# zhu-xlab/PFST

Measured on AMD Instinct MI355X. Metric: PFST train-step images/s on 1024² IRRG tiles, higher is better.
Workload: dtype f32 (f16x3 split MFMA: two scaled fp16 pieces per operand, three products, fp32 accumulate); 1 GPU; pfst_pots_irrg2vaih_irrg_deeplabv3plus_r50-d8; global_batch=8, per_gpu_batch=8, tile=1024x1024x3, num_classes=6, parallelism=dp1, weights=seeded random init, conv_math=f16x3

## Files before the change

### pfst_amd/csrc/conv_f16x3.hip

```cpp
#include "conv_epilogue.h"
#include "amax.h"
#include "wgrad_launch.h"
#include "weight_jobs.h"
#include <math.h>
#include <stdlib.h>
#include <type_traits>
#include <utility>
#include "../../include/pfst_hip.h"

typedef _Float16 f16x8 __attribute__((ext_vector_type(8)));
typedef float f32x4 __attribute__((ext_vector_type(4)));

namespace {

constexpr int BN = 128;
constexpr int NP = 2;

__global__ __launch_bounds__(256) void absmax_kernel(const float* __restrict__ x, i64 n, i64 plane_stride, int slot_stride,
                                                     float* __restrict__ slots) {
  const float* p = x + (i64)blockIdx.y * plane_stride;
  float m = 0.f;
  const i64 n4 = (((uintptr_t)p & 15) == 0) ? n / 4 : 0;
  for (i64 i = (i64)blockIdx.x * blockDim.x + threadIdx.x; i < n4; i += (i64)gridDim.x * blockDim.x) {
    const float4 v = reinterpret_cast<const float4*>(p)[i];
// ... 218 lines not shown
    if constexpr (ONE) {
      ld_oy = p;
      ld_ox = 0;
    } else {
      ld_oy = ld_pvalid ? p / Wo : 0;
      ld_ox = ld_pvalid ? p - ld_oy * Wo : 0;
    }
    a_voff = (m0 + a_row < M) ? 16u * ((unsigned)a_seg * (unsigned)M + (unsigned)(m0 + a_row)) : OOB;
    a_rsrc = __builtin_amdgcn_make_buffer_rsrc(const_cast<uint4*>(wk4) + (i64)y * KT16 * 2 * NP * M, 0, KT16 * 2 * NP * M * 16, 0x00020000);
    b_rsrc = __builtin_amdgcn_make_buffer_rsrc(const_cast<float*>(in) + (i64)n * in_bs, 0, C * HiWi * 4, 0x00020000);
  };
  auto tap_voff = [&](int tap) -> unsigned {
    if constexpr (ONE) return ld_pvalid ? 4u * ((unsigned)(bt * 16 + kh * 8) * (unsigned)HiWi + (unsigned)ld_oy) : OOB;
    const int ty = tap / ks, tx = tap - ty * ks;
    int sy, sx;
    const bool ok = ld_pvalid & src_coord(ld_oy, ty, ca, cb, cc, cdivv, Hi, sy) & src_coord(ld_ox, tx, ca, cb, cc, cdivv, Wi, sx);
    return ok ? 4u * ((unsigned)(kh * 8) * (unsigned)HiWi + (unsigned)(sy * Wi + sx)) : OOB;
  };

  uint4 areg[2][NA];
  float breg[2][TPT][8];
  pfst_f32x16 acc32[TMW][2];
#pragma unroll
  for (int i = 0; i < TMW; ++i)
#pragma unroll
    for (int j = 0; j < 2; ++j)
#pragma unroll
      for (int r = 0; r < 16; ++r) acc32[i][j][r] = 0.f;

  auto load_b = [&](auto vc, auto setc, unsigned voff, int soff) {
    constexpr int v = decltype(vc)::value, SET = decltype(setc)::value;
    breg[SET][v >> 3][v & 7] = __builtin_bit_cast(float, __builtin_amdgcn_raw_buffer_load_b32(b_rsrc, voff, soff + ((v >> 3) * 16 + (v & 7)) * b_chan, 0));
  };
  auto load_a = [&](auto vc, auto setc, int a_soff) {
    constexpr int v = decltype(vc)::value, SET = decltype(setc)::value;
    areg[SET][v] = __builtin_bit_cast(uint4, __builtin_amdgcn_raw_buffer_load_b128(a_rsrc, a_voff, a_soff + (v / (NA / 2)) * a_tile + (v % (NA / 2)) * a_chunk, 0));
  };
  int tap2 = 0, sidx2 = 0;
  int sidx1 = 0;
  unsigned voff2 = OOB;
  auto advance = [&]() {
    sidx1 = sidx2;
    if (++sidx2 == spt) {
      sidx2 = 0;
      ++tap2;
      if (tap2 < ntaps) {
        voff2 = tap_voff(tap2);
      } else if (CHAIN && tap2 == ntaps && ld_lin + G < total) {
        ld_lin += G;
        set_load_side(ld_lin);
        tap2 = 0;
        voff2 = tap_voff(0);
      } else {
        voff2 = OOB;
      }
    }
  };

  const int eb = amax_exponent(amax_read(in_amax));
  const float sb = __builtin_bit_cast(float, __builtin_amdgcn_readfirstlane(__builtin_bit_cast(int, scale_of(eb))));
  int ea = 0, ea_y = -1;

  auto prologue = [&](int lin) {
    ld_lin = lin;
    set_load_side(lin);
    tap2 = sidx2 = 0;
    voff2 = tap_voff(0);
    static_for<8 * TPT>([&](auto vc) { load_b(vc, std::integral_constant<int, 0>(), voff2, 0); });
    static_for<NA>([&](auto vc) { load_a(vc, std::integral_constant<int, 0>(), 0); });
    advance();
#pragma unroll
    for (int v = 0; v < NA; ++v) As[(v / (NA / 2)) * TILE_A + tid + NT * (v % (NA / 2))] = areg[0][v];
#pragma unroll
    for (int t = 0; t < TPT; ++t) {
      uint4 ph, pl;
      if constexpr (BNL) {
        const float2* cf = reinterpret_cast<const float2*>(bnl_s) + (t + bt) * 16 + kh * 8;
#pragma unroll
        for (int i = 0; i < 8; ++i) breg[0][t][i] = fmaxf(__fmaf_rn(breg[0][t][i], cf[i].x, cf[i].y), 0.f);
      }
      if constexpr (BPACK) unpack8_f16(breg[0][t], ph, pl);
      else split8_f16(breg[0][t], sb, ph, pl);
      Bs[(t + bt) * TILE_B + (0 * 2 + kh) * BN + pix] = ph;
      Bs[(t + bt) * TILE_B + (1 * 2 + kh) * BN + pix] = pl;
    }
    {
      const int soff = sidx2 * chan_step, a_soff = (tap2 * spt + sidx2) * 2 * a_tile;
      static_for<8 * TPT>([&](auto vc) { load_b(vc, std::integral_constant<int, 1>(), voff2, soff); });
      static_for<NA>([&](auto vc) { load_a(vc, std::integral_constant<int, 1>(), a_soff); });
    }
    advance();
    __syncthreads();
  };

  const int l15 = lane & 15, lq = lane >> 4;
  const int a_frag = (lq >> 1) * TILE_A + (lq & 1) * BM + wm0 + l15;
  const int b_frag = (lq >> 1) * TILE_B + (lq & 1) * BN + wn0 + l15;

  const int l31 = lane & 31, lh = lane >> 5;
  auto step32 = [&](auto setn_c, int k) {
    constexpr int SETN = decltype(setn_c)::value, SETL = SETN ^ 1;
    constexpr int CUR = SETL * PAIR_CHUNKS, NXT = SETN * PAIR_CHUNKS;
    f16x8 af[2][TMW][NP], bf[2][2][NP];
    auto rd_a = [&](int t, int i, int pl) { af[t][i][pl] = __builtin_bit_cast(f16x8, As[CUR + t * TILE_A + (pl * 2 + lh) * BM + wm0 + i * 32 + l31]); };
    auto rd_b = [&](int t, int j, int pl) { bf[t][j][pl] = __builtin_bit_cast(f16x8, Bs[CUR + t * TILE_B + (pl * 2 + lh) * BN + wn0 + j * 32 + l31]); };
    constexpr int RG = 2 + TMW;
    auto read_frag = [&](auto rc) {
      constexpr int r = decltype(rc)::value, grp = r / RG, e = r % RG, t = grp & 1, pa = grp < 2 ? 1 : 0, pb = grp < 2 ? 0 : 1;
      if constexpr (e == 0) rd_a(t, 0, pa);
      else if constexpr (e == 1) rd_b(t, 0, pb);
      else if constexpr (e == 2) rd_b(t, 1, pb);
      else rd_a(t, 1, pa);
    };
    const int soff2 = sidx2 * chan_step;
    const int a_soff2 = (tap2 * spt + sidx2) * 2 * a_tile;
    constexpr int PRE = TMW == 2 ? RG : 2 * RG;
    static_for<PRE>([&](auto rc) { read_frag(rc); });
    __builtin_amdgcn_sched_barrier(0);
    SplitF16 s0, s1;
    uint4 cfr[BNL ? 4 : 1];
    const int cf_at = BNL ? sidx1 * 16 + bt * 8 + kh * 4 : 0;
    auto filler = [&](auto sc) {
      constexpr int m = decltype(sc)::value;
      if constexpr (m < 8) {
        if constexpr (TPT == 2) {
          load_b(std::integral_constant<int, 2 * m>(), std::integral_constant<int, SETL>(), voff2, soff2);
          load_b(std::integral_constant<int, 2 * m + 1>(), std::integral_constant<int, SETL>(), voff2, soff2);
        } else {
          load_b(std::integral_constant<int, m>(), std::integral_constant<int, SETL>(), voff2, soff2);
        }
      }
      if constexpr (m >= 8 && m < 8 + NA) As[NXT + ((m - 8) / (NA / 2)) * TILE_A + tid + NT * ((m - 8) % (NA / 2))] = areg[SETN][m - 8];
      if constexpr (BNL && m >= 8 && m < 12) cfr[m - 8] = bnl_s[cf_at + (m - 8)];
      if constexpr (m >= 12) {
        constexpr int SPS = 2 * TPT;
        static_for<SPS>([&](auto kc) {
          constexpr int kk = (m - 12) * SPS + decltype(kc)::value;
          if constexpr (BPACK) {
            if constexpr (kk < 8) unpack_op_f16<kk>(breg[SETN][0], s0);
            else if constexpr (kk < 16 && TPT == 2) unpack_op_f16<kk - 8>(breg[SETN][TPT - 1], s1);
          } else {
            if constexpr (BNL && kk < 24 && kk % 6 < 2) {
              constexpr int e = 2 * (kk / 6) + kk % 6;
              const uint4 c2 = cfr[e >> 1];
              const float sc = __builtin_bit_cast(float, (e & 1) ? c2.z : c2.x), sh = __builtin_bit_cast(float, (e & 1) ? c2.w : c2.y);
              breg[SETN][0][e] = fmaxf(__fmaf_rn(breg[SETN][0][e], sc, sh), 0.f);
            }
            if constexpr (kk < 24) split_op_f16<kk>(breg[SETN][0], sb, s0);
            else split_op_f16<kk - 24>(breg[SETN][TPT - 1], sb, s1);
          }
        });
      }
      if constexpr (m >= 12 && m < 12 + NA) load_a(std::integral_constant<int, m - 12>(), std::integral_constant<int, SETL>(), a_soff2);
      if constexpr (m == 18 && TPT == 2) {
        Bs[NXT + (0 * 2 + kh) * BN + pix] = make_uint4(s0.h[0], s0.h[1], s0.h[2], s0.h[3]);
        Bs[NXT + (1 * 2 + kh) * BN + pix] = make_uint4(s0.l[0], s0.l[1], s0.l[2], s0.l[3]);
      }
      if constexpr (m == 23 && TPT == 2) {
        Bs[NXT + TILE_B + (0 * 2 + kh) * BN + pix] = make_uint4(s1.h[0], s1.h[1], s1.h[2], s1.h[3]);
        Bs[NXT + TILE_B + (1 * 2 + kh) * BN + pix] = make_uint4(s1.l[0], s1.l[1], s1.l[2], s1.l[3]);
      }
      if constexpr (m == 23 && TPT == 1) {
        Bs[NXT + bt * TILE_B + (0 * 2 + kh) * BN + pix] = make_uint4(s0.h[0], s0.h[1], s0.h[2], s0.h[3]);
        Bs[NXT + bt * TILE_B + (1 * 2 + kh) * BN + pix] = make_uint4(s0.l[0], s0.l[1], s0.l[2], s0.l[3]);
      }
    };
    static_for<12 * TMW>([&](auto mc) {
      constexpr int m = decltype(mc)::value;
      constexpr int prod = m / (4 * TMW), rem = m % (4 * TMW), t = rem / (2 * TMW), i = (rem >> 1) % TMW, j = rem & 1;
      constexpr int pa = prod == 0 ? 1 : 0, pb = prod == 1 ? 1 : 0;
      acc32[i][j] = __builtin_amdgcn_mfma_f32_32x32x16_f16(af[t][i][pa], bf[t][j][pb], acc32[i][j], 0, 0, 0);
      if constexpr (PRE + m < 4 * RG) read_frag(std::integral_constant<int, PRE + m>());
      if constexpr (TMW == 2) {
        filler(std::integral_constant<int, m>());
      } else {
        filler(std::integral_constant<int, 2 * m>());
        filler(std::integral_constant<int, 2 * m + 1>());
      }
      __builtin_amdgcn_sched_barrier(0);
    });
    advance();
    __syncthreads();
  };
  auto epilogue = [&](int lin) {
    int bx, by, y, n;
    decode(lin, bx, by, y, n);
    if (y != ea_y) {
      ea = amax_exponent(amax_read(w_amax + (i64)y * PFST_AMAX_SUB));
      ea_y = y;
    }
    const int p0 = bx * BN, m0 = by * BM;
    float* const outn = out + (i64)n * out_bs;
    const float* const gsrc = gate.g ? gate.g + (i64)n * gate.g_bs : nullptr;
    const unsigned long long* const gmask = gate.g ? gate.mask + (i64)n * M * (P >> 6) : nullptr;
    const float ua = unscale_of(ea), ub = unscale_of(eb);
    {
#pragma unroll
      for (int i = 0; i < TMW; ++i)
#pragma unroll
        for (int j = 0; j < 2; ++j)
#pragma unroll
          for (int r = 0; r < 16; ++r) acc32[i][j][r] = acc32[i][j][r] * ua * ub;
      if constexpr (BNB != 0) {
        static_assert(PAIR_CHUNKS * sizeof(uint4) >= (NT / 64) * PFST_ROWSUM_LDS_FLOATS * sizeof(float), "epilogue scratch must fit into one pair buffer");
        conv_epilogue<2, 2, WAVES_N, BN, BNB, true>(acc32, outn, bias, stats, stats_T, accumulate, M, P, m0, p0, wm0, wn0, bx, n, wid, lane, bnb,
                                                    reinterpret_cast<float*>(smem + PAIR_CHUNKS), gsrc, gmask, nullptr, nt_out);
        __syncthreads();
      } else {
#ifdef PFST_STATS_LDSRED
        if (stats && !stats_mm && BMT != 64) {
          conv_epilogue<TMW, 2, WAVES_N, BN, 0, true>(acc32, outn, bias, stats, stats_T, accumulate, M, P, m0, p0, wm0, wn0, bx, n, wid, lane, PfstBnbArgs(),
                                                      reinterpret_cast<float*>(smem + PAIR_CHUNKS), gsrc, gmask, nullptr, nt_out);
          __syncthreads();
        } else
#endif
        conv_epilogue<TMW, 2, WAVES_N, BN>(acc32, outn, bias, stats, stats_T, accumulate, M, P, m0, p0, wm0, wn0, bx, n, wid, lane, PfstBnbArgs(), nullptr,
                                           gsrc, gmask, stats_mm, nt_out);
      }
#pragma unroll
      for (int i = 0; i < TMW; ++i)
#pragma unroll
        for (int j = 0; j < 2; ++j)
#pragma unroll
          for (int r = 0; r < 16; ++r) acc32[i][j][r] = 0.f;
    }
  };

  for (int lin = blockIdx.x; lin < total; lin += G) {
    if (!CHAIN || lin == (int)blockIdx.x) prologue(lin);
    for (int k = 0; k < KP; k += 2) {
      step32(std::integral_constant<int, 1>(), k);
      if (k + 1 < KP) step32(std::integral_constant<int, 0>(), k + 1);
    }
    epilogue(lin);
  }
}

template <int SHAPE, bool BPACK = false, bool ONE = false, int BMT = 128>
__global__ __launch_bounds__(BMT == 64 ? 256 : 2 * BMT, BMT == 256 ? 1 : 2) void conv_igemm_f16x3_kernel(
    const float* __restrict__ in, i64 in_bs, const uint4* __restrict__ wk4, const float* __restrict__ bias,
    float* __restrict__ out, i64 out_bs, int C, int Hi, int Wi, int M, int Ho, int Wo, int ks,
    int ca, int cb, int cc, int cdivv, int accumulate, float* __restrict__ stats, int stats_T,
    const float* __restrict__ w_amax, const float* __restrict__ in_amax, int Y, int Z, int chain, PfstResGate gate) {
  conv_igemm_f16x3_body<SHAPE, 0, BPACK, ONE, BMT>(in, in_bs, wk4, bias, out, out_bs, C, Hi, Wi, M, Ho, Wo, ks, ca, cb, cc, cdivv, accumulate, stats, stats_T,
                               w_amax, in_amax, Y, Z, chain, PfstBnbArgs(), gate);
}
__global__ __launch_bounds__(512, 1) void conv_igemm_f16x3_bnl_kernel(
    const float* __restrict__ in, i64 in_bs, const uint4* __restrict__ wk4, const float* __restrict__ bias,
    float* __restrict__ out, i64 out_bs, int C, int Hi, int Wi, int M, int Ho, int Wo, int ks,
    int ca, int cb, int cc, int cdivv, int accumulate, float* __restrict__ stats, int stats_T,
    const float* __restrict__ w_amax, const float* __restrict__ in_amax, int Y, int Z, int chain, const float4* __restrict__ bnl) {
  conv_igemm_f16x3_body<32, 0, false, true, 256, true>(in, in_bs, wk4, bias, out, out_bs, C, Hi, Wi, M, Ho, Wo, ks, ca, cb, cc, cdivv, accumulate, stats,
                                                       stats_T, w_amax, in_amax, Y, Z, chain, PfstBnbArgs(), PfstResGate(), bnl);
}
template <int BNB, bool ONE = false, int BMT = 128>
__global__ __launch_bounds__(2 * BMT, BMT == 128 ? 2 : 1) void conv_igemm_f16x3_bnb_kernel(
    const float* __restrict__ in, i64 in_bs, const uint4* __restrict__ wk4, const float* __restrict__ bias,
    float* __restrict__ out, i64 out_bs, int C, int Hi, int Wi, int M, int Ho, int Wo, int ks,
    int ca, int cb, int cc, int cdivv, int accumulate, float* __restrict__ stats, int stats_T,
    const float* __restrict__ w_amax, const float* __restrict__ in_amax, int Y, int Z, int chain, PfstBnbArgs bnb, PfstResGate gate) {
  conv_igemm_f16x3_body<32, BNB, false, ONE, BMT>(in, in_bs, wk4, bias, out, out_bs, C, Hi, Wi, M, Ho, Wo, ks, ca, cb, cc, cdivv, accumulate, stats, stats_T,
                                 w_amax, in_amax, Y, Z, chain, bnb, gate);
}


typedef float f32x16 __attribute__((ext_vector_type(16)));

struct Split4 {
  unsigned h[2], l[2];
  float t0[2], t1[2];
};
#ifdef PFST_F16X3_SPLIT6
template <int K>
__device__ __forceinline__ void split4_op_f16(const float (&v)[4], float s, Split4& st) {
  constexpr int q = K / 6, op = K % 6;
  if constexpr (op == 0) asm volatile("v_mul_f32 %0, %1, %2" : "=v"(st.t0[q]) : "s"(s), "v"(v[2 * q]));
  else if constexpr (op == 1) asm volatile("v_mul_f32 %0, %1, %2" : "=v"(st.t1[q]) : "s"(s), "v"(v[2 * q + 1]));
  else if constexpr (op == 2) asm volatile("v_cvt_pk_f16_f32 %0, %1, %2" : "=v"(st.h[q]) : "v"(st.t0[q]), "v"(st.t1[q]));
  else if constexpr (op == 3)
    asm volatile("v_fma_mix_f32 %0, %1, %2, -%3 op_sel:[0,0,0] op_sel_hi:[0,0,1]" : "=v"(st.t0[q]) : "v"(v[2 * q]), "s"(s), "v"(st.h[q]));
  else if constexpr (op == 4)
    asm volatile("v_fma_mix_f32 %0, %1, %2, -%3 op_sel:[0,0,1] op_sel_hi:[0,0,1]" : "=v"(st.t1[q]) : "v"(v[2 * q + 1]), "s"(s), "v"(st.h[q]));
  else asm volatile("v_cvt_pk_f16_f32 %0, %1, %2" : "=v"(st.l[q]) : "v"(st.t0[q]), "v"(st.t1[q]));
}
#else
template <int K>
__device__ __forceinline__ void split4_op_f16(const float (&v)[4], float s, Split4& st) {
  constexpr int q = K / 6, op = K % 6;
  if constexpr (op == 2) asm volatile("v_fma_mixlo_f16 %0, %1, %2, 0 op_sel_hi:[0,0,0]" : "=v"(st.h[q]) : "v"(v[2 * q]), "s"(s));
  else if constexpr (op == 3) asm volatile("v_fma_mixhi_f16 %0, %1, %2, 0 op_sel_hi:[0,0,0]" : "+v"(st.h[q]) : "v"(v[2 * q + 1]), "s"(s));
  else if constexpr (op == 4)
    asm volatile("v_fma_mixlo_f16 %0, %1, %2, -%3 op_sel:[0,0,0] op_sel_hi:[0,0,1]" : "=v"(st.l[q]) : "v"(v[2 * q]), "s"(s), "v"(st.h[q]));
  else if constexpr (op == 5)
    asm volatile("v_fma_mixhi_f16 %0, %1, %2, -%3 op_sel:[0,0,1] op_sel_hi:[0,0,1]" : "+v"(st.l[q]) : "v"(v[2 * q + 1]), "s"(s), "v"(st.h[q]));
}
#endif
template <int K>
__device__ __forceinline__ void unpack4_op_f16(const float (&v)[4], Split4& st) {
  constexpr int q = K & 1;
  if constexpr (K < 2) asm volatile("v_perm_b32 %0, %1, %2, %3" : "=v"(st.h[q]) : "v"(v[2 * q + 1]), "v"(v[2 * q]), "s"(0x05040100u));
  else asm volatile("v_perm_b32 %0, %1, %2, %3" : "=v"(st.l[q]) : "v"(v[2 * q + 1]), "v"(v[2 * q]), "s"(0x07060302u));
}

template <bool PACK, int BMT = 128, bool BNL = false>
__global__ __launch_bounds__(2 * BMT, BMT == 128 ? 2 : 1) void conv_wgrad_f16x3_line_kernel(
    const float* __restrict__ x, i64 x_bs, const float* __restrict__ dy, i64 dy_bs, float* __restrict__ dw,
    int J, int M, int P, int chunks, int chunk_len, int N, i64 x_gs, i64 dy_gs, i64 dw_gs, int gx, int gy, int gz,
    const float* __restrict__ x_amax, const float* __restrict__ dy_amax, const float4* __restrict__ bnl) {
  static_assert(!BNL || !PACK, "a pre-split operand is already normalised");
  constexpr int BM = BMT, BJ = 128, WM = 64, WAVES_N = 2, WN = 64, TM = 2, TN = 2, NT = 2 * BM;
  constexpr int RPP = NT / 8;
  constexpr int PA = BM / RPP, PB = BJ / RPP;
  constexpr int ROWS_A = BM + 2, ROWS_B = BJ + 2;
  constexpr int TILE_A = 4 * ROWS_A + 4, TILE_B = 4 * ROWS_B + 4;
  __shared__ uint4 As[2][2 * TILE_A];
  __shared__ uint4 Bs[2][2 * TILE_B];

  const int tid = threadIdx.x, lane = tid & 63, wid = __builtin_amdgcn_readfirstlane(tid >> 6);
  const int wm0 = (wid / WAVES_N) * WM, wn0 = (wid % WAVES_N) * WN;
  int bx, by, bz;
  {
    const int lin = blockIdx.x, tiles = gx * gy, z8 = gz & ~7;
    if (lin < tiles * z8) {
      const int xcd = lin & 7, idx = lin >> 3;
      const int sl = idx / tiles, t = idx - sl * tiles;
      bz = sl * 8 + xcd;
      by = t / gx;
      bx = t - by * gx;
    } else {
      bz = lin / tiles;
      const int t = lin - bz * tiles;
      by = t / gx;
      bx = t - by * gx;
    }
  }
  const int j0 = bx * BJ, m0 = by * BM;
  const int ng = bz / chunks, chunk = bz - ng * chunks;
  const int grp = ng / N, n = ng - grp * N;
  const int pbeg = chunk * chunk_len;
  const int pend = min(P, pbeg + chunk_len);
  if (pbeg >= pend) return;
  x += (i64)grp * x_gs + (i64)n * x_bs;
  dy += (i64)grp * dy_gs + (i64)n * dy_bs;
  dw += dw_gs >= 0 ? (i64)grp * dw_gs : (i64)bz * -dw_gs;
  const int ea = amax_exponent(amax_read(dy_amax)), eb = amax_exponent(amax_read(x_amax));
  const float sa = __builtin_bit_cast(float, __builtin_amdgcn_readfirstlane(__builtin_bit_cast(int, scale_of(ea))));
  const float sb = __builtin_bit_cast(float, __builtin_amdgcn_readfirstlane(__builtin_bit_cast(int, scale_of(eb))));
  const __amdgpu_buffer_rsrc_t a_rsrc = __builtin_amdgcn_make_buffer_rsrc(const_cast<float*>(dy), 0, M * P * 4, 0x00020000);
  const __amdgpu_buffer_rsrc_t b_rsrc = __builtin_amdgcn_make_buffer_rsrc(const_cast<float*>(x), 0, J * P * 4, 0x00020000);

  const int rslot = tid >> 3, seg = tid & 7;
  constexpr unsigned OOB = 0x80000000u;
  const unsigned a_voff = 4u * ((unsigned)(m0 + rslot) * (unsigned)P) + 16u * seg;
  const unsigned b_voff = 4u * ((unsigned)(j0 + rslot) * (unsigned)P) + 16u * seg;
  const int row_step = RPP * P * 4;
  const int a_half = 2 * ((seg >> 2) * TILE_A + ((seg >> 1) & 1) * ROWS_A + rslot) + (seg & 1);
  const int b_half = 2 * ((seg >> 2) * TILE_B + ((seg >> 1) & 1) * ROWS_B + rslot) + (seg & 1);

  float la[2][PA][4], lb[2][PB][4];
  float bsc[BNL ? PB : 1], bsh[BNL ? PB : 1];
  if constexpr (BNL) {
#pragma unroll
    for (int p = 0; p < PB; ++p) {
      const int j = j0 + rslot + p * RPP;
      const float4 cf = j < J ? bnl[j] : make_float4(0.f, 0.f, 0.f, 0.f);
      bsc[p] = cf.z;
      bsh[p] = cf.w;
    }
  }
  auto normalise = [&](float (&v)[4], int p) {
#pragma unroll
    for (int e = 0; e < 4; ++e) v[e] = fmaxf(__fmaf_rn(v[e], bsc[p], bsh[p]), 0.f);
  };
  f32x16 acc[TM][TN];
#pragma unroll
  for (int i = 0; i < TM; ++i)
#pragma unroll
    for (int j = 0; j < TN; ++j)
#pragma unroll
      for (int r = 0; r < 16; ++r) acc[i][j][r] = 0.f;

  auto load_quad = [&](auto qc, auto setc, int pk0) {
    constexpr int q = decltype(qc)::value, SET = decltype(setc)::value, opb = q >= PA, pass = opb ? q - PA : q;
    const bool v = pk0 + 4 * seg < pend;
    const float4 w = __builtin_bit_cast(float4, __builtin_amdgcn_raw_buffer_load_b128(opb ? b_rsrc : a_rsrc, v ? (opb ? b_voff : a_voff) : OOB,
                                                                                      pk0 * 4 + pass * row_step, 0));
    float (&dst)[4] = opb ? lb[SET][pass] : la[SET][pass];
    dst[0] = w.x; dst[1] = w.y; dst[2] = w.z; dst[3] = w.w;
  };
  auto store_half = [&](auto qc, int buf, const Split4& st) {
    constexpr int q = decltype(qc)::value, opb = q >= PA, pass = opb ? q - PA : q;
    if constexpr (opb) {
      uint2* b2 = reinterpret_cast<uint2*>(&Bs[buf][0]);
      b2[b_half + 2 * pass * RPP] = make_uint2(st.h[0], st.h[1]);
      b2[b_half + 2 * (pass * RPP + 2 * ROWS_B)] = make_uint2(st.l[0], st.l[1]);
    } else {
      uint2* a2 = reinterpret_cast<uint2*>(&As[buf][0]);
      a2[a_half + 2 * pass * RPP] = make_uint2(st.h[0], st.h[1]);
      a2[a_half + 2 * (pass * RPP + 2 * ROWS_A)] = make_uint2(st.l[0], st.l[1]);
    }
  };
  const int l31 = lane & 31, lh = lane >> 5;

  static_for<PA + PB>([&](auto qc) { load_quad(qc, std::integral_constant<int, 0>(), pbeg); });
  static_for<PA + PB>([&](auto qc) {
    constexpr int q = decltype(qc)::value, opb = q >= PA, pass = opb ? q - PA : q;
    Split4 st;
    if constexpr (BNL && opb) normalise(lb[0][pass], pass);
    static_for<PACK ? 4 : 12>([&](auto kc) {
      if constexpr (PACK) unpack4_op_f16<decltype(kc)::value>(opb ? lb[0][pass] : la[0][pass], st);
      else split4_op_f16<decltype(kc)::value>(opb ? lb[0][pass] : la[0][pass], opb ? sb : sa, st);
    });
    store_half(qc, 0, st);
  });
  static_for<PA + PB>([&](auto qc) { load_quad(qc, std::integral_constant<int, 1>(), pbeg + 32); });
  __syncthreads();

  auto step = [&](auto curc, int kp) {
    constexpr int CUR = decltype(curc)::value, NXT = CUR ^ 1;
    f16x8 af[2][TM][NP], bf[2][TN][NP];
    auto rd_a = [&](int t, int i, int pl) { af[t][i][pl] = __builtin_bit_cast(f16x8, As[CUR][t * TILE_A + (pl * 2 + lh) * ROWS_A + wm0 + i * 32 + l31]); };
    auto rd_b = [&](int t, int j, int pl) { bf[t][j][pl] = __builtin_bit_cast(f16x8, Bs[CUR][t * TILE_B + (pl * 2 + lh) * ROWS_B + wn0 + j * 32 + l31]); };
    auto read_frag = [&](auto rc) {
      constexpr int r = decltype(rc)::value, grp = r >> 2, e = r & 3, t = grp & 1, pa = grp < 2 ? 1 : 0, pb = grp < 2 ? 0 : 1;
      if constexpr (e == 0) rd_a(t, 0, pa);
      else if constexpr (e == 1) rd_b(t, 0, pb);
      else if constexpr (e == 2) rd_b(t, 1, pb);
      else rd_a(t, 1, pa);
    };
    static_for<4>([&](auto rc) { read_frag(rc); });
    __builtin_amdgcn_sched_barrier(0);
    Split4 st[2];
    const int pk2 = pbeg + (kp + 2) * 32;
    static_for<24>([&](auto mc) {
      constexpr int m = decltype(mc)::value;
      constexpr int prod = m >> 3, t = (m >> 2) & 1, i = (m >> 1) & 1, j = m & 1;
      constexpr int pa = prod == 0 ? 1 : 0, pb = prod == 1 ? 1 : 0;
      acc[i][j] = __builtin_amdgcn_mfma_f32_32x32x16_f16(af[t][i][pa], bf[t][j][pb], acc[i][j], 0, 0, 0);
      if constexpr (m < 12) read_frag(std::integral_constant<int, 4 + m>());
      if constexpr (m < PA + PB) load_quad(mc, curc, pk2);
      constexpr int q = m / 3, part = m % 3;
      if constexpr (q < PA + PB) {
        constexpr int opb = q >= PA, pass = opb ? q - PA : q;
        if constexpr (BNL && opb && part == 0) normalise(lb[NXT][pass], pass);
        static_for<4>([&](auto kc) {
          constexpr int k = part * 4 + decltype(kc)::value;
          if constexpr (PACK) {
            if constexpr (k < 4) unpack4_op_f16<k>(opb ? lb[NXT][pass] : la[NXT][pass], st[q & 1]);
          } else {
            split4_op_f16<k>(opb ? lb[NXT][pass] : la[NXT][pass], opb ? sb : sa, st[q & 1]);
          }
        });
        if constexpr (part == 2) store_half(std::integral_constant<int, q>(), NXT, st[q & 1]);
      }
      __builtin_amdgcn_sched_barrier(0);
    });
    __syncthreads();
  };
  const int KPAIRS = (pend - pbeg + 31) / 32;
  for (int kp = 0; kp < KPAIRS; kp += 2) {
    step(std::integral_constant<int, 0>(), kp);
    if (kp + 1 < KPAIRS) step(std::integral_constant<int, 1>(), kp + 1);
  }
  const float ua = unscale_of(ea), ub = unscale_of(eb);
#pragma unroll
  for (int i = 0; i < TM; ++i) {
#pragma unroll
    for (int j = 0; j < TN; ++j) {
      const int jj = j0 + wn0 + j * 32 + l31;
#pragma unroll
      for (int r = 0; r < 16; ++r) {
        const int m = m0 + wm0 + i * 32 + (r & 3) + 8 * (r >> 2) + 4 * lh;
        if (m < M && jj < J) atomicAdd(&dw[(i64)m * J + jj], acc[i][j][r] * ua * ub);
      }
    }
  }
}

int f16x3_slots_override = 0;
unsigned f16x3_grid(i64 total, bool chainable, int wg_per_cu = 2) {
  static int cus = 0;
  if (cus == 0) {
    int dev = 0;
    if (hipGetDevice(&dev) != hipSuccess || hipDeviceGetAttribute(&cus, hipDeviceAttributeMultiprocessorCount, dev) != hipSuccess || cus <= 0) cus = 256;
  }
  int slots = (f16x3_slots_override > 0 ? f16x3_slots_override : 2 * cus) * wg_per_cu / 2;
  if (slots < 1) slots = 1;
  if (!chainable || total <= slots) return (unsigned)total;
  i64 best_g = total;
  double best_waste = 1e30;
  for (int t = 0; t <= 32; ++t) {
    const i64 g = t == 0 ? slots : (total + t - 1) / t;
    if (g < slots) continue;
    const i64 per_wg = (total + g - 1) / g, rounds = (g + slots - 1) / slots;
    if (per_wg > 8) continue;
    const double waste = (double)(rounds * per_wg * slots) / (double)total;
    if (waste < best_waste - 1e-9 || (waste < best_waste + 1e-9 && g < best_g)) { best_waste = waste; best_g = g; }
  }
  return (unsigned)best_g;
}


}

extern "C" int pfst_f16x3_set_slots(int slots) {
  PFST_CHECK_ARG(slots >= 0);
  f16x3_slots_override = slots;
  return PFST_OK;
}

extern "C" int pfst_f16x3_chain_grid(long long total_tiles, int chainable) {
  if (total_tiles <= 0 || total_tiles >= (1ll << 31)) return 0;
  return (int)f16x3_grid(total_tiles, chainable != 0);
}

namespace {
__global__ __launch_bounds__(256) void f16x3_split_probe_kernel(const float* __restrict__ x, i64 n8, const float* __restrict__ amax,
                                                                unsigned* __restrict__ pieces_loop, unsigned* __restrict__ pieces_loop4,
                                                                unsigned* __restrict__ pieces_plain) {
  const float s = __builtin_bit_cast(float, __builtin_amdgcn_readfirstlane(__builtin_bit_cast(int, scale_of(amax_exponent(amax_read(amax))))));
  for (i64 g = (i64)blockIdx.x * blockDim.x + threadIdx.x; g < n8; g += (i64)gridDim.x * blockDim.x) {
    float v[8];
#pragma unroll
    for (int j = 0; j < 8; ++j) v[j] = x[g * 8 + j];
    SplitF16 st;
    static_for<24>([&](auto kc) { split_op_f16<decltype(kc)::value>(v, s, st); });
    uint4 ph, pl;
    split8_f16(v, s, ph, pl);
    const unsigned hp[4] = {ph.x, ph.y, ph.z, ph.w}, lp[4] = {pl.x, pl.y, pl.z, pl.w};
#pragma unroll
    for (int q = 0; q < 4; ++q) {
      pieces_loop[g * 8 + 2 * q] = (st.h[q] & 0xffffu) | (st.l[q] << 16);
      pieces_loop[g * 8 + 2 * q + 1] = (st.h[q] >> 16) | (st.l[q] & 0xffff0000u);
      pieces_plain[g * 8 + 2 * q] = (hp[q] & 0xffffu) | (lp[q] << 16);
      pieces_plain[g * 8 + 2 * q + 1] = (hp[q] >> 16) | (lp[q] & 0xffff0000u);
    }
#pragma unroll
    for (int half = 0; half < 2; ++half) {
      const float v4[4] = {v[4 * half], v[4 * half + 1], v[4 * half + 2], v[4 * half + 3]};
      Split4 s4;
      static_for<12>([&](auto kc) { split4_op_f16<decltype(kc)::value>(v4, s, s4); });
#pragma unroll
      for (int q = 0; q < 2; ++q) {
        pieces_loop4[g * 8 + 4 * half + 2 * q] = (s4.h[q] & 0xffffu) | (s4.l[q] << 16);
        pieces_loop4[g * 8 + 4 * half + 2 * q + 1] = (s4.h[q] >> 16) | (s4.l[q] & 0xffff0000u);
      }
    }
  }
}
}

extern "C" int pfst_f16x3_split_probe(const float* x, long long n, const float* amax, unsigned* pieces_loop, unsigned* pieces_loop4,
                                      unsigned* pieces_plain, pfst_stream_t stream) {
  PFST_CHECK_ARG(x && amax && pieces_loop && pieces_loop4 && pieces_plain && n > 0 && n % 8 == 0);
  hipLaunchKernelGGL(f16x3_split_probe_kernel, dim3(ew_grid(n / 8)), dim3(256), 0, (hipStream_t)stream, x, (i64)(n / 8), amax, pieces_loop,
                     pieces_loop4, pieces_plain);
  PFST_CHECK_LAUNCH();
  return PFST_OK;
}

extern "C" int pfst_absmax(const float* x, long long n, int planes, long long plane_stride, int slot_stride, float* slots,
                           pfst_stream_t stream) {
  PFST_CHECK_ARG(x && slots && n > 0 && planes > 0 && planes <= 65535 && (slot_stride == 0 || slot_stride == 1));
  int gx = (int)((n / 4 + 255) / 256);
  if (gx < 1) gx = 1;
  const int cap = planes > 1 ? 256 : 2048;
  if (gx > cap) gx = cap;
  hipLaunchKernelGGL(absmax_kernel, dim3(gx, planes), dim3(256), 0, (hipStream_t)stream, x, (i64)n, (i64)plane_stride, slot_stride, slots);
  PFST_CHECK_LAUNCH();
  return PFST_OK;
}

extern "C" int pfst_conv_pack_weight_f16x2(const float* w, void* wk4_fprop, void* wk4_dgrad, int Cout, int Cin, int T, int sets,
                                           const float* amax, pfst_stream_t stream) {
  PFST_CHECK_ARG(w && amax && (wk4_fprop || wk4_dgrad) && Cout > 0 && Cin > 0 && (T == 1 || T == 9) && sets >= 1 && sets <= 65535);
  PFST_CHECK_ARG(!wk4_fprop || Cin % 16 == 0);
  PFST_CHECK_ARG(!wk4_dgrad || Cout % 16 == 0);
  PFST_CHECK_ARG(sets == 1 || T == 1);
  const i64 n = (i64)Cout * Cin * T;
  int gx = ew_grid(n / 8 + 1);
  if (gx > 4096) gx = 4096;
  hipLaunchKernelGGL(pack_weight_f16x2_kernel, dim3(gx, sets), dim3(256), 0, (hipStream_t)stream, w, (uint4*)wk4_fprop, (uint4*)wk4_dgrad,
                     Cout, Cin, T, n, 4 * n / 16, amax);
  PFST_CHECK_LAUNCH();
  return PFST_OK;
}

extern "C" int pfst_conv_pack_weight_f16x2_batched(const pfst_weight_job_t* jobs_host, const pfst_weight_job_t* jobs_dev, int njobs,
                                                   pfst_stream_t stream) {
  PFST_CHECK_ARG(jobs_host && jobs_dev && njobs > 0);
  i64 blocks = 0;
  for (int j = 0; j < njobs; ++j) {
    const pfst_weight_job_t& J = jobs_host[j];
    PFST_CHECK_ARG(J.src && J.amax_f && (J.dst_f || J.dst_d) && J.Cout > 0 && J.Cin > 0 && (J.T == 1 || J.T == 9) && J.sets >= 1);
    PFST_CHECK_ARG((!J.dst_f || J.Cin % 16 == 0) && (!J.dst_d || J.Cout % 16 == 0) && (J.sets == 1 || J.T == 1) && J.first_block == blocks);
    blocks += weight_job_blocks(J, 1);
  }
  PFST_CHECK_ARG(blocks < (1ll << 31));
  hipLaunchKernelGGL(pack_weight_f16x2_batched_kernel, dim3((unsigned)blocks), dim3(256), 0, (hipStream_t)stream, jobs_dev, njobs);
  PFST_CHECK_LAUNCH();
  return PFST_OK;
}

extern "C" int pfst_conv_igemm_f16x3(const float* in, long long in_bs, const void* wk4, const float* w_amax, const float* in_amax,
                                     const float* bias, float* out, long long out_bs, int N, int C, int Hi, int Wi, int M, int Ho, int Wo,
                                     int ksize, int stride, int dil, int pad, int mode, int accumulate, float* stats,
                                     const pfst_bnb_fuse_t* bnb, const float* gate_dy, long long gate_dy_bs,
                                     const unsigned long long* gate_mask, int stats_minmax, const float* bnl, pfst_stream_t stream) {
  PFST_CHECK_ARG(in && wk4 && w_amax && in_amax && out && N > 0 && C > 0 && M > 0 && Hi > 0 && Wi > 0 && Ho > 0 && Wo > 0);
  PFST_CHECK_ARG(!bnl || (mode == 0 && ksize == 1 && stride == 1 && pad == 0 && M % 256 == 0 && C <= 2048 && !bias && !gate_dy && !(bnb && bnb->x) &&
                          !accumulate));
  PFST_CHECK_ARG(!stats_minmax || (stats && !bias && !(bnb && bnb->x)));
  PfstResGate gate;
  if (gate_dy) {
    PFST_CHECK_ARG(gate_mask && mode == 1 && !accumulate && !bias && !stats && M % 128 == 0 && ((i64)Ho * Wo) % 256 == 0 &&
                   gate_dy_bs >= (i64)M * Ho * Wo);
    gate.g = gate_dy;
    gate.g_bs = gate_dy_bs;
    gate.mask = gate_mask;
  }
  PFST_CHECK_ARG(!bnb || (bnb->x && bnb->x_bs >= (i64)M * Ho * Wo && (!bnb->y || bnb->y_bs >= (i64)M * Ho * Wo)));
  PFST_CHECK_ARG(!bnb || !bnb->y_mask || (bnb->y && bnb->relu && ((i64)Ho * Wo) % 256 == 0));
  ConvGeom g;
  if (const int rc = conv_geometry(Hi, Wi, Ho, Wo, ksize, stride, dil, pad, mode, g)) return rc;
  PFST_CHECK_ARG(in_bs >= (i64)C * Hi * Wi && out_bs >= (i64)M * Ho * Wo && N <= 65535);
  PFST_CHECK_ARG((i64)C * Hi * Wi * 4 < (1ll << 31) && (i64)M * Ho * Wo * 4 < (1ll << 31) && (i64)ksize * ksize * C * M * 4 < (1ll << 31));
  if ((C % 32 != 0 && !(ksize == 1 && C % 16 == 0)) || M <= 32) {
    pfst_set_error(__FILE__, __LINE__, "f16x3 kernel needs C % 32 == 0 (1x1: C % 16 == 0) and more than 32 output channels (use pfst_conv_igemm_split)");
    return PFST_ERR_UNSUPPORTED;
  }
  const bool small = M <= 64;
  PFST_CHECK_ARG(!small || !(bnb && bnb->x));
  const int a = g.a, b = g.b, c = g.c, d = g.d;
  const int stats_T = N * (int)cdiv((i64)Ho * Wo, BN) * 2;
  const bool one = !small && ksize == 1 && stride == 1 && pad == 0;
  const bool big = one && M % 256 == 0;
  const i64 total = (i64)cdiv((i64)Ho * Wo, BN) * cdiv(M, big ? 256 : small ? 64 : 128) * N;
  PFST_CHECK_ARG(total < (1ll << 31));
  const dim3 grid(f16x3_grid(total, one && ((C + 31) / 32) % 2 == 0, big ? 1 : 2));
  const int chain = 1 | (stats_minmax ? 2 : 0) | 4;
  if (bnb && bnb->x) {
    PFST_CHECK_ARG(M % 128 == 0 && !bias && !stats && bnb->coef && bnb->partials);
#define PFST_LAUNCH_F16_BNB(KERNEL_, THREADS_)                                                                                              \
    hipLaunchKernelGGL(KERNEL_, grid, dim3(THREADS_), 0, (hipStream_t)stream, in, (i64)in_bs, (const uint4*)wk4, bias, out, (i64)out_bs, C, Hi, Wi, \
                       M, Ho, Wo, ksize, a, b, c, d, accumulate, stats, stats_T, w_amax, in_amax, 1, N, chain, *bnb, gate)
    with_bnb_mode<true>(*bnb, [&](auto mode) {
      constexpr int MODE = decltype(mode)::value;
      if (big) PFST_LAUNCH_F16_BNB((conv_igemm_f16x3_bnb_kernel<MODE, true, 256>), 512);
      else if (one) PFST_LAUNCH_F16_BNB((conv_igemm_f16x3_bnb_kernel<MODE, true>), 256);
      else PFST_LAUNCH_F16_BNB((conv_igemm_f16x3_bnb_kernel<MODE, false>), 256);
    });
#undef PFST_LAUNCH_F16_BNB
    PFST_CHECK_LAUNCH();
    return PFST_OK;
  }
  if (bnl)
    hipLaunchKernelGGL(conv_igemm_f16x3_bnl_kernel, grid, dim3(512), 0, (hipStream_t)stream, in, (i64)in_bs, (const uint4*)wk4, bias, out, (i64)out_bs, C, Hi, Wi,
                       M, Ho, Wo, ksize, a, b, c, d, accumulate, stats, stats_T, w_amax, in_amax, 1, N, chain, reinterpret_cast<const float4*>(bnl));
  else if (small)
    hipLaunchKernelGGL((conv_igemm_f16x3_kernel<32, false, false, 64>), grid, dim3(256), 0, (hipStream_t)stream, in, (i64)in_bs, (const uint4*)wk4, bias, out,
                       (i64)out_bs, C, Hi, Wi, M, Ho, Wo, ksize, a, b, c, d, accumulate, stats, stats_T, w_amax, in_amax, 1, N, chain, gate);
  else if (big)
    hipLaunchKernelGGL((conv_igemm_f16x3_kernel<32, false, true, 256>), grid, dim3(512), 0, (hipStream_t)stream, in, (i64)in_bs, (const uint4*)wk4, bias, out,
                       (i64)out_bs, C, Hi, Wi, M, Ho, Wo, ksize, a, b, c, d, accumulate, stats, stats_T, w_amax, in_amax, 1, N, chain, gate);
  else if (one)
    hipLaunchKernelGGL((conv_igemm_f16x3_kernel<32, false, true>), grid, dim3(256), 0, (hipStream_t)stream, in, (i64)in_bs, (const uint4*)wk4, bias, out,
                       (i64)out_bs, C, Hi, Wi, M, Ho, Wo, ksize, a, b, c, d, accumulate, stats, stats_T, w_amax, in_amax, 1, N, chain, gate);
  else
    hipLaunchKernelGGL(conv_igemm_f16x3_kernel<32>, grid, dim3(256), 0, (hipStream_t)stream, in, (i64)in_bs, (const uint4*)wk4, bias, out,
                       (i64)out_bs, C, Hi, Wi, M, Ho, Wo, ksize, a, b, c, d, accumulate, stats, stats_T, w_amax, in_amax, 1, N, chain, gate);
  PFST_CHECK_LAUNCH();
  return PFST_OK;
}

extern "C" int pfst_wino_gemm_f16x3(const float* V, const void* U4, const float* u_amax, const float* v_amax, float* Mbuf, int N, int K,
                                    int M, int T, int m, int v_packed, pfst_stream_t stream) {
  PFST_CHECK_ARG(V && U4 && u_amax && v_amax && Mbuf && N > 0 && N <= 65535 && K > 0 && K % 32 == 0 && M > 64 && T > 0 && (m == 2 || m == 4));
  const int nx = (m + 2) * (m + 2);
  PFST_CHECK_ARG((i64)K * T * 4 < (1ll << 31) && (i64)M * T * 4 < (1ll << 31) && (i64)K * M * 4 < (1ll << 31));
  const bool big = M % 256 == 0;
  const i64 total = (i64)cdiv((i64)T, BN) * cdiv(M, big ? 256 : 128) * nx * N;
  PFST_CHECK_ARG(total < (1ll << 31));
  const dim3 grid(f16x3_grid(total, (K / 32) % 2 == 0, big ? 1 : 2));
  const int chain = 1 | 4;
  if (big && v_packed)
    hipLaunchKernelGGL((conv_igemm_f16x3_kernel<32, true, true, 256>), grid, dim3(512), 0, (hipStream_t)stream, V, (i64)K * T, (const uint4*)U4,
                       (const float*)nullptr, Mbuf, (i64)M * T, K, 1, T, M, 1, T, 1, 1, 1, 0, 1, 0, (float*)nullptr, 0, u_amax, v_amax, nx, N, chain, PfstResGate());
  else if (big)
    hipLaunchKernelGGL((conv_igemm_f16x3_kernel<32, false, true, 256>), grid, dim3(512), 0, (hipStream_t)stream, V, (i64)K * T, (const uint4*)U4,
                       (const float*)nullptr, Mbuf, (i64)M * T, K, 1, T, M, 1, T, 1, 1, 1, 0, 1, 0, (float*)nullptr, 0, u_amax, v_amax, nx, N, chain, PfstResGate());
  else if (v_packed)
    hipLaunchKernelGGL((conv_igemm_f16x3_kernel<32, true, true>), grid, dim3(256), 0, (hipStream_t)stream, V, (i64)K * T, (const uint4*)U4,
                       (const float*)nullptr, Mbuf, (i64)M * T, K, 1, T, M, 1, T, 1, 1, 1, 0, 1, 0, (float*)nullptr, 0, u_amax, v_amax, nx, N, chain, PfstResGate());
  else
    hipLaunchKernelGGL((conv_igemm_f16x3_kernel<32, false, true>), grid, dim3(256), 0, (hipStream_t)stream, V, (i64)K * T, (const uint4*)U4, (const float*)nullptr,
                       Mbuf, (i64)M * T, K, 1, T, M, 1, T, 1, 1, 1, 0, 1, 0, (float*)nullptr, 0, u_amax, v_amax, nx, N, chain, PfstResGate());
  PFST_CHECK_LAUNCH();
  return PFST_OK;
}

int pfst_wgrad_f16x3_launch(const float* x, i64 x_bs, const float* dy, i64 dy_bs, float* dw, int N, int J, int M, int P, int groups,
                            i64 x_gs, i64 dy_gs, i64 dw_gs, const float* x_amax, const float* dy_amax, int packed, hipStream_t s, const float* bnl) {
  PFST_CHECK_ARG(!bnl || (!packed && groups == 1));
  const float4* const bnl4 = reinterpret_cast<const float4*>(bnl);
  const bool big = M % 256 == 0;
  const int bm = big ? 256 : 128;
  const int tiles = cdiv(J, 128) * cdiv(M, bm) * groups;
  const SplitK k = plan_split_k((i64)tiles * N, P, big ? 256 : 256 * 2, 16);
  const int gx = cdiv(J, 128), gy = cdiv(M, bm), gz = N * groups * k.chunks;
  PFST_CHECK_ARG((i64)gx * gy * gz < (1ll << 31));
  return wgrad_launch(dw, (i64)M * J, groups, N * k.chunks, dw_gs, s, [&](float* dst, i64 group_stride, i64) {
#define PFST_LAUNCH_WGRAD(KERNEL_, THREADS_)                                                                                               \
  hipLaunchKernelGGL(KERNEL_, dim3(gx * gy * gz), dim3(THREADS_), 0, s, x, x_bs, dy, dy_bs, dst, J, M, P, k.chunks, k.chunk_len, N, x_gs, dy_gs, \
                     group_stride, gx, gy, gz, x_amax, dy_amax, bnl4)
    if (bnl && big) PFST_LAUNCH_WGRAD((conv_wgrad_f16x3_line_kernel<false, 256, true>), 512);
    else if (bnl) PFST_LAUNCH_WGRAD((conv_wgrad_f16x3_line_kernel<false, 128, true>), 256);
    else if (big && packed) PFST_LAUNCH_WGRAD((conv_wgrad_f16x3_line_kernel<true, 256>), 512);
    else if (big) PFST_LAUNCH_WGRAD((conv_wgrad_f16x3_line_kernel<false, 256>), 512);
    else if (packed) PFST_LAUNCH_WGRAD((conv_wgrad_f16x3_line_kernel<true>), 256);
    else PFST_LAUNCH_WGRAD((conv_wgrad_f16x3_line_kernel<false>), 256);
#undef PFST_LAUNCH_WGRAD
  });
}

extern "C" int pfst_conv_wgrad_f16x3(const float* x, long long x_bs, const float* dy, long long dy_bs, float* dw, int N, int Cin, int Cout,
                                     int HW, const float* x_amax, const float* dy_amax, const float* bnl, pfst_stream_t stream) {
  PFST_CHECK_ARG(x && dy && dw && x_amax && dy_amax && N > 0 && Cin > 0 && Cout > 0 && HW > 0);
  PFST_CHECK_ARG(x_bs >= (i64)Cin * HW && dy_bs >= (i64)Cout * HW && (x_bs & 3) == 0 && (dy_bs & 3) == 0);
  PFST_CHECK_ARG((((uintptr_t)x | (uintptr_t)dy) & 15) == 0 && (i64)Cin * HW * 4 < (1ll << 31) && (i64)Cout * HW * 4 < (1ll << 31));
  if (HW % 4 != 0 || Cout <= 64) {
    pfst_set_error(__FILE__, __LINE__, "f16x3 weight gradient needs HW % 4 == 0 and more than 64 output channels (use pfst_conv_wgrad_split)");
    return PFST_ERR_UNSUPPORTED;
  }
  return pfst_wgrad_f16x3_launch(x, x_bs, dy, dy_bs, dw, N, Cin, Cout, HW, 1, 0, 0, 0, x_amax, dy_amax, 0, (hipStream_t)stream, bnl);
}
```

Baseline: 29.61 images/s.

## Peel full K-steps, prefetch next fragments early, and lean wgrad epilogue

Splits the wgrad K loop into a bounds-check-free body of whole steps followed by a guarded tail. It also moves the first LDS fragment reads of the next step ahead of the barrier so they overlap the MFMA tail. For interior tiles the atomic epilogue skips the per-element bounds checks. Diagnostic timestamp and ablation macros are added but are off by default. The early read changes where the barrier sits and raises register pressure.

Measured after the change: 29.75 images/s, median of 6. About the same (+0.5%).

```diff
diff --git a/pfst_amd/csrc/conv_f16x3.hip b/pfst_amd/csrc/conv_f16x3.hip
--- a/pfst_amd/csrc/conv_f16x3.hip
+++ b/pfst_amd/csrc/conv_f16x3.hip
@@ -544,6 +544,22 @@
   else asm volatile("v_perm_b32 %0, %1, %2, %3" : "=v"(st.l[q]) : "v"(v[2 * q + 1]), "v"(v[2 * q]), "s"(0x07060302u));
 }
 
+#ifndef PFST_WGRAD_DIAG
+#define PFST_WGRAD_DIAG 0
+#endif
+#ifndef PFST_WGRAD_PEEL
+#define PFST_WGRAD_PEEL 1
+#endif
+#ifndef PFST_WGRAD_EARLY
+#define PFST_WGRAD_EARLY 1
+#endif
+#ifndef PFST_WGRAD_LEAN_EPILOGUE
+#define PFST_WGRAD_LEAN_EPILOGUE 1
+#endif
+#ifdef PFST_WGRAD_STAMPS
+constexpr int WGRAD_STAMP_WGS = 256, WGRAD_STAMP_N = 8;
+__device__ unsigned long long wgrad_stamps[WGRAD_STAMP_WGS * 8 * WGRAD_STAMP_N];
+#endif
 template <bool PACK, int BMT = 128, bool BNL = false>
 __global__ __launch_bounds__(2 * BMT, BMT == 128 ? 2 : 1) void conv_wgrad_f16x3_line_kernel(
     const float* __restrict__ x, i64 x_bs, const float* __restrict__ dy, i64 dy_bs, float* __restrict__ dw,
@@ -611,8 +627,10 @@
     }
   }
   auto normalise = [&](float (&v)[4], int p) {
-#pragma unroll
-    for (int e = 0; e < 4; ++e) v[e] = fmaxf(__fmaf_rn(v[e], bsc[p], bsh[p]), 0.f);
+    if constexpr ((PFST_WGRAD_DIAG & 8) == 0) {
+#pragma unroll
+      for (int e = 0; e < 4; ++e) v[e] = fmaxf(__fmaf_rn(v[e], bsc[p], bsh[p]), 0.f);
+    }
   };
   f32x16 acc[TM][TN];
 #pragma unroll
@@ -622,11 +640,11 @@
 #pragma unroll
       for (int r = 0; r < 16; ++r) acc[i][j][r] = 0.f;
 
-  auto load_quad = [&](auto qc, auto setc, int pk0) {
+  auto load_quad = [&](auto qc, auto setc, int pk0, auto wholec) {
     constexpr int q = decltype(qc)::value, SET = decltype(setc)::value, opb = q >= PA, pass = opb ? q - PA : q;
-    const bool v = pk0 + 4 * seg < pend;
-    const float4 w = __builtin_bit_cast(float4, __builtin_amdgcn_raw_buffer_load_b128(opb ? b_rsrc : a_rsrc, v ? (opb ? b_voff : a_voff) : OOB,
-                                                                                      pk0 * 4 + pass * row_step, 0));
+    unsigned voff = opb ? b_voff : a_voff;
+    if constexpr (!decltype(wholec)::value && (PFST_WGRAD_DIAG & 4) == 0) voff = pk0 + 4 * seg < pend ? voff : OOB;
+    const float4 w = __builtin_bit_cast(float4, __builtin_amdgcn_raw_buffer_load_b128(opb ? b_rsrc : a_rsrc, voff, pk0 * 4 + pass * row_step, 0));
     float (&dst)[4] = opb ? lb[SET][pass] : la[SET][pass];
     dst[0] = w.x; dst[1] = w.y; dst[2] = w.z; dst[3] = w.w;
   };
@@ -644,33 +662,86 @@
   };
   const int l31 = lane & 31, lh = lane >> 5;
 
-  static_for<PA + PB>([&](auto qc) { load_quad(qc, std::integral_constant<int, 0>(), pbeg); });
+  auto split_op = [&](auto kc, auto opbc, const float (&v)[4], Split4& st) {
+    constexpr int k = decltype(kc)::value, opb = decltype(opbc)::value;
+    if constexpr ((PFST_WGRAD_DIAG & (opb ? 1 : 2)) != 0) {
+      if constexpr (k == 3) {
+        st.h[0] = __builtin_bit_cast(unsigned, v[0]); st.l[0] = __builtin_bit_cast(unsigned, v[1]);
+        st.h[1] = __builtin_bit_cast(unsigned, v[2]); st.l[1] = __builtin_bit_cast(unsigned, v[3]);
+      }
+    } else if constexpr (PACK) {
+      if constexpr (k < 4) unpack4_op_f16<k>(v, st);
+    } else {
+      split4_op_f16<k>(v, opb ? sb : sa, st);
+    }
+  };
+  const int KPAIRS = (pend - pbeg + 31) / 32;
+  const int KWHOLE = PFST_WGRAD_PEEL ? max((pend - pbeg) / 32 - 2, 0) & ~1 : 0;
+  const std::true_type whole_c;
+  const std::false_type part_c;
+
+  if (KWHOLE > 0) {
+    static_for<PA + PB>([&](auto qc) { load_quad(qc, std::integral_constant<int, 0>(), pbeg, whole_c); });
+  } else {
+    static_for<PA + PB>([&](auto qc) { load_quad(qc, std::integral_constant<int, 0>(), pbeg, part_c); });
+  }
   static_for<PA + PB>([&](auto qc) {
     constexpr int q = decltype(qc)::value, opb = q >= PA, pass = opb ? q - PA : q;
     Split4 st;
     if constexpr (BNL && opb) normalise(lb[0][pass], pass);
-    static_for<PACK ? 4 : 12>([&](auto kc) {
-      if constexpr (PACK) unpack4_op_f16<decltype(kc)::value>(opb ? lb[0][pass] : la[0][pass], st);
-      else split4_op_f16<decltype(kc)::value>(opb ? lb[0][pass] : la[0][pass], opb ? sb : sa, st);
-    });
+    static_for<12>([&](auto kc) { split_op(kc, std::integral_constant<int, opb>(), opb ? lb[0][pass] : la[0][pass], st); });
     store_half(qc, 0, st);
   });
-  static_for<PA + PB>([&](auto qc) { load_quad(qc, std::integral_constant<int, 1>(), pbeg + 32); });
+  if (KWHOLE > 0) {
+    static_for<PA + PB>([&](auto qc) { load_quad(qc, std::integral_constant<int, 1>(), pbeg + 32, whole_c); });
+  } else {
+    static_for<PA + PB>([&](auto qc) { load_quad(qc, std::integral_constant<int, 1>(), pbeg + 32, part_c); });
+  }
   __syncthreads();
 
-  auto step = [&](auto curc, int kp) {
+#ifdef PFST_WGRAD_STAMPS
+  auto stamp = [&]() {
+    unsigned long long t;
+    __builtin_amdgcn_sched_barrier(0);
+    asm volatile("s_memtime %0\n\ts_waitcnt lgkmcnt(0)" : "=s"(t) : : "memory");
+    __builtin_amdgcn_sched_barrier(0);
+    return t;
+  };
+  unsigned long long s_head = 0, s_vm = 0, s_tail = 0, s_bar = 0, s_steps = 0;
+#endif
+  constexpr bool EARLY = PFST_WGRAD_EARLY && 3 * (PA + PB) <= 20 && (PFST_WGRAD_DIAG & 16) == 0;
+  f16x8 af[2][TM][NP], bf[2][TN][NP];
+  auto read_frag = [&](auto rc, auto bufc) {
+    constexpr int r = decltype(rc)::value, BUF = decltype(bufc)::value, grp = r >> 2, e = r & 3, t = grp & 1, pa = grp < 2 ? 1 : 0, pb = grp < 2 ? 0 : 1;
+    constexpr int i = e == 0 ? 0 : 1, j = e == 1 ? 0 : 1;
+    if constexpr (e == 0 || e == 3) af[t][i][pa] = __builtin_bit_cast(f16x8, As[BUF][t * TILE_A + (pa * 2 + lh) * ROWS_A + wm0 + i * 32 + l31]);
+    else bf[t][j][pb] = __builtin_bit_cast(f16x8, Bs[BUF][t * TILE_B + (pb * 2 + lh) * ROWS_B + wn0 + j * 32 + l31]);
+  };
+  if constexpr (EARLY) static_for<4>([&](auto rc) { read_frag(rc, std::integral_constant<int, 0>()); });
+  auto step_barrier = [&]() {
+#ifdef PFST_WGRAD_STAMPS
+    const unsigned long long t0 = stamp(), t1 = stamp();
+    __syncthreads();
+    const unsigned long long t2 = stamp();
+    s_tail += t1 - t0;
+    s_bar += t2 - t1;
+#else
+    if constexpr ((PFST_WGRAD_DIAG & 16) == 0) __syncthreads();
+#endif
+  };
+  auto step = [&](auto curc, int kp, auto wholec) {
     constexpr int CUR = decltype(curc)::value, NXT = CUR ^ 1;
-    f16x8 af[2][TM][NP], bf[2][TN][NP];
-    auto rd_a = [&](int t, int i, int pl) { af[t][i][pl] = __builtin_bit_cast(f16x8, As[CUR][t * TILE_A + (pl * 2 + lh) * ROWS_A + wm0 + i * 32 + l31]); };
-    auto rd_b = [&](int t, int j, int pl) { bf[t][j][pl] = __builtin_bit_cast(f16x8, Bs[CUR][t * TILE_B + (pl * 2 + lh) * ROWS_B + wn0 + j * 32 + l31]); };
-    auto read_frag = [&](auto rc) {
-      constexpr int r = decltype(rc)::value, grp = r >> 2, e = r & 3, t = grp & 1, pa = grp < 2 ? 1 : 0, pb = grp < 2 ? 0 : 1;
-      if constexpr (e == 0) rd_a(t, 0, pa);
-      else if constexpr (e == 1) rd_b(t, 0, pb);
-      else if constexpr (e == 2) rd_b(t, 1, pb);
-      else rd_a(t, 1, pa);
-    };
-    static_for<4>([&](auto rc) { read_frag(rc); });
+    if constexpr (!EARLY) static_for<4>([&](auto rc) { read_frag(rc, curc); });
+#ifdef PFST_WGRAD_STAMPS
+    {
+      const unsigned long long t0 = stamp(), t1 = stamp();
+      asm volatile("s_waitcnt vmcnt(0)" : : : "memory");
+      const unsigned long long t2 = stamp();
+      s_head += t1 - t0;
+      s_vm += t2 - t1;
+      s_steps += 1;
+    }
+#endif
     __builtin_amdgcn_sched_barrier(0);
     Split4 st[2];
     const int pk2 = pbeg + (kp + 2) * 32;
@@ -679,45 +750,80 @@
       constexpr int prod = m >> 3, t = (m >> 2) & 1, i = (m >> 1) & 1, j = m & 1;
       constexpr int pa = prod == 0 ? 1 : 0, pb = prod == 1 ? 1 : 0;
       acc[i][j] = __builtin_amdgcn_mfma_f32_32x32x16_f16(af[t][i][pa], bf[t][j][pb], acc[i][j], 0, 0, 0);
-      if constexpr (m < 12) read_frag(std::integral_constant<int, 4 + m>());
-      if constexpr (m < PA + PB) load_quad(mc, curc, pk2);
+      if constexpr (m < 12) read_frag(std::integral_constant<int, 4 + m>(), curc);
+      if constexpr (EARLY && m >= 20) read_frag(std::integral_constant<int, m - 20>(), std::integral_constant<int, NXT>());
+      if constexpr (m < PA + PB) load_quad(mc, curc, pk2, wholec);
       constexpr int q = m / 3, part = m % 3;
       if constexpr (q < PA + PB) {
         constexpr int opb = q >= PA, pass = opb ? q - PA : q;
         if constexpr (BNL && opb && part == 0) normalise(lb[NXT][pass], pass);
         static_for<4>([&](auto kc) {
-          constexpr int k = part * 4 + decltype(kc)::value;
-          if constexpr (PACK) {
-            if constexpr (k < 4) unpack4_op_f16<k>(opb ? lb[NXT][pass] : la[NXT][pass], st[q & 1]);
-          } else {
-            split4_op_f16<k>(opb ? lb[NXT][pass] : la[NXT][pass], opb ? sb : sa, st[q & 1]);
-          }
+          split_op(std::integral_constant<int, part * 4 + decltype(kc)::value>(), std::integral_constant<int, opb>(), opb ? lb[NXT][pass] : la[NXT][pass],
+                   st[q & 1]);
         });
         if constexpr (part == 2) store_half(std::integral_constant<int, q>(), NXT, st[q & 1]);
       }
+      if constexpr (EARLY && m == 3 * (PA + PB) - 1) step_barrier();
       __builtin_amdgcn_sched_barrier(0);
     });
-    __syncthreads();
-  };
-  const int KPAIRS = (pend - pbeg + 31) / 32;
-  for (int kp = 0; kp < KPAIRS; kp += 2) {
-    step(std::integral_constant<int, 0>(), kp);
-    if (kp + 1 < KPAIRS) step(std::integral_constant<int, 1>(), kp + 1);
-  }
+    if constexpr (!EARLY) step_barrier();
+  };
+#ifdef PFST_WGRAD_STAMPS
+  const unsigned long long loop_t0 = stamp();
+#endif
+  int kp = 0;
+  for (; kp < KWHOLE; kp += 2) {
+    step(std::integral_constant<int, 0>(), kp, whole_c);
+    step(std::integral_constant<int, 1>(), kp + 1, whole_c);
+  }
+  for (; kp < KPAIRS; kp += 2) {
+    step(std::integral_constant<int, 0>(), kp, part_c);
+    if (kp + 1 < KPAIRS) step(std::integral_constant<int, 1>(), kp + 1, part_c);
+  }
+#ifdef PFST_WGRAD_STAMPS
+  {
+    const unsigned long long loop_t1 = stamp();
+    if (lane == 0 && blockIdx.x < WGRAD_STAMP_WGS && wid < 8) {
+      unsigned long long* o = &wgrad_stamps[((int)blockIdx.x * 8 + wid) * WGRAD_STAMP_N];
+      o[0] = s_head; o[1] = s_vm; o[2] = s_tail; o[3] = s_bar; o[4] = loop_t1 - loop_t0; o[5] = s_steps; o[6] = 0; o[7] = 0;
+    }
+  }
+#endif
   const float ua = unscale_of(ea), ub = unscale_of(eb);
-#pragma unroll
-  for (int i = 0; i < TM; ++i) {
-#pragma unroll
-    for (int j = 0; j < TN; ++j) {
-      const int jj = j0 + wn0 + j * 32 + l31;
-#pragma unroll
-      for (int r = 0; r < 16; ++r) {
-        const int m = m0 + wm0 + i * 32 + (r & 3) + 8 * (r >> 2) + 4 * lh;
-        if (m < M && jj < J) atomicAdd(&dw[(i64)m * J + jj], acc[i][j][r] * ua * ub);
-      }
-    }
-  }
-}
+  const unsigned lane_off = (unsigned)(4 * lh * J + l31);
+  auto add_tile = [&](auto wholec) {
+#pragma unroll
+    for (int i = 0; i < TM; ++i) {
+#pragma unroll
+      for (int j = 0; j < TN; ++j) {
+        const int jj = j0 + wn0 + j * 32 + l31;
+#pragma unroll
+        for (int r = 0; r < 16; ++r) {
+          const int mu = m0 + wm0 + i * 32 + (r & 3) + 8 * (r >> 2);
+          const float v = acc[i][j][r] * ua * ub;
+          if constexpr ((PFST_WGRAD_DIAG & 32) != 0) {
+            if (v != 1.2345e-30f) continue;
+          }
+          if constexpr (decltype(wholec)::value) atomicAdd(dw + ((i64)mu * J + (j0 + wn0 + j * 32)) + lane_off, v);
+          else if (mu + 4 * lh < M && jj < J) atomicAdd(&dw[(i64)(mu + 4 * lh) * J + jj], v);
+        }
+      }
+    }
+  };
+  if (PFST_WGRAD_LEAN_EPILOGUE && m0 + BM <= M && j0 + BJ <= J) add_tile(whole_c);
+  else add_tile(part_c);
+}
+
+#ifdef PFST_WGRAD_STAMPS
+}
+extern "C" int pfst_wgrad_read_stamps(unsigned long long* host, int n) {
+  PFST_CHECK_ARG(host && n > 0 && n <= WGRAD_STAMP_WGS * 8 * WGRAD_STAMP_N);
+  if (hipDeviceSynchronize() != hipSuccess) return PFST_ERR_LAUNCH;
+  if (hipMemcpyFromSymbol(host, HIP_SYMBOL(wgrad_stamps), n * sizeof(unsigned long long)) != hipSuccess) return PFST_ERR_LAUNCH;
+  return PFST_OK;
+}
+namespace {
+#endif
 
 int f16x3_slots_override = 0;
 unsigned f16x3_grid(i64 total, bool chainable, int wg_per_cu = 2) {
```
